# Cyan4973/FiniteStateEntropy

Measured on NVIDIA H100. Metric: encode+decode GB/s (uncompressed) per GPU on 32 KB blocks; bit-exact vs ref, higher is better.
Workload: dtype u8

## Files before the change

finitestateentropy_b200/csrc/huf_encode.cu:

```cuda
#include <cstdlib>
#include <mutex>
#include <type_traits>
#include <vector>
#include "common.cuh"
#include "launchers.h"
#include "launch_util.cuh"
#include "fse_dev.cuh"
#include "sink_dev.cuh"
#include "huf_build_dev.cuh"
#include "pack_dev.cuh"

namespace fseb {
namespace hufe {

constexpr unsigned FULL = 0xFFFFFFFFu;

struct __align__(16) Plan {
    u32 ctable[256];
    u8  header[136];
    u32 hSize;
    u32 state;
    u32 total;
    u32 streamOff[4];
    u32 streamBytes[4];
    u16 segCount[4][256];
};

constexpr int PLAN_WARPS = 8;
constexpr u32 GROUP = 32;
constexpr u32 HDR_STRIDE = 34 + 224 + 1;
constexpr u32 CT_ROW = HDR_STRIDE;
constexpr u32 ROWS = CT_ROW + 256;
constexpr u32 NODE_END = 0x7FFFFFFFu, LEAF_END = 0xFFFFFFFFu;
struct PlanCta {
    u32 nd[ROWS][GROUP];
    u8  sym[256][GROUP];
    u64 res[GROUP];
    u16 msv[GROUP];
    u8  last[GROUP];
    u8  tlog[GROUP];
    u8  live[GROUP];
};
static_assert(ROWS >= 1 + 256 + PLAN_WARPS * 4 * 256 / GROUP, "segment histograms must fit in the rows above the leaves");
static_assert(ROWS >= 1 + 511 && CT_ROW >= 1 + 256, "node rows");
static_assert(HUF_BLOCK_MAX < (1u << 24), "node counts share a word with an 8-bit parent / length");
static_assert(sizeof(PlanCta) <= 76 * 1024, "three CTAs per SM");

__device__ __forceinline__ void warp_hist_range(u32* cnt, const u8* s, u32 begin, u32 end, unsigned lane)
{
    u32 i = begin;
    u32 const head = min(end, (u32)((begin + 15) & ~15u));
    bool const vec = ((reinterpret_cast<u64>(s) & 15) == 0);
    if (vec) {
        for (u32 k = i + lane; k < head; k += 32) atomicAdd(&cnt[s[k]], 1u);
        i = head;
        u32 const nvec = (end - i) / 16;
        const uint4* const gv = reinterpret_cast<const uint4*>(s + i);
        for (u32 v0 = 0; v0 < nvec; v0 += 128) {
            uint4 x[4];
            #pragma unroll
            for (int h = 0; h < 4; h++) { u32 const vi = v0 + 32 * h + lane; x[h] = (vi < nvec) ? __ldg(gv + vi) : make_uint4(0, 0, 0, 0); }
            #pragma unroll
            for (int h = 0; h < 4; h++) {
                if (v0 + 32 * h + lane >= nvec) continue;
                u32 const wd[4] = { x[h].x, x[h].y, x[h].z, x[h].w };
                #pragma unroll
                for (int k = 0; k < 4; k++) {
                    u32 const y = wd[k];
                    atomicAdd(&cnt[y & 0xFF], 1u); atomicAdd(&cnt[__byte_perm(y, 0, 0x4441)], 1u);
                    atomicAdd(&cnt[__byte_perm(y, 0, 0x4442)], 1u); atomicAdd(&cnt[y >> 24], 1u);
                }
            }
        }
        i += nvec * 16;
    }
    for (u32 k = i + lane; k < end; k += 32) atomicAdd(&cnt[s[k]], 1u);
}

__device__ __forceinline__ void warp_hist4_pipelined(u32 (*count4)[256], const u8* s, u32 n, u32 seg, unsigned lane)
{
    const uint4* const gv = reinterpret_cast<const uint4*>(s) + lane;
    u32 const B = n / 2048, perSeg = seg / 2048;
    auto load = [&](uint4 (&x)[4], u32 b) {
        #pragma unroll
        for (int h = 0; h < 4; h++) x[h] = __ldg(gv + b * 128 + 32 * h);
    };
    auto count = [&](const uint4 (&x)[4], u32 b) {
        u32* const cnt = count4[b / perSeg];
        #pragma unroll
        for (int h = 0; h < 4; h++) {
            u32 const wd[4] = { x[h].x, x[h].y, x[h].z, x[h].w };
            #pragma unroll
            for (int k = 0; k < 4; k++) {
                u32 const y = wd[k];
                atomicAdd(&cnt[y & 0xFF], 1u); atomicAdd(&cnt[__byte_perm(y, 0, 0x4441)], 1u);
                atomicAdd(&cnt[__byte_perm(y, 0, 0x4442)], 1u); atomicAdd(&cnt[y >> 24], 1u);
            }
        }
    };
    uint4 xa[4], xb[4];
    load(xa, 0);
    #pragma unroll 1
    for (u32 b = 0; b < B; b += 2) {
        if (b + 1 < B) load(xb, b + 1);
        count(xa, b);
        if (b + 2 < B) load(xa, b + 2);
        if (b + 1 < B) count(xb, b + 1);
    }
}

template <class Geo, int NS>
__global__ void __launch_bounds__(32 * PLAN_WARPS, 3)
huf_plan_kernel(Geo g, u8* __restrict__ cbuf, u64* __restrict__ csizes, const u8* __restrict__ src,
                unsigned msvReq, unsigned tlogReq, Plan* __restrict__ plans)
{
    static_assert(NS == 4 || NS == 1, "4X or 1X");
    extern __shared__ __align__(16) unsigned char smem_raw[];
    PlanCta& S = *reinterpret_cast<PlanCta*>(smem_raw);
    unsigned const lane = threadIdx.x & 31u, warp = threadIdx.x >> 5;
    u32 const b0 = blockIdx.x * GROUP;
#define FSEB_FINAL(v) { if (lane == 0) { P.state = 1; enc_out(g, csizes, b) = (v); S.live[c] = 0; } continue; }

    u32 (*const count4)[256] = reinterpret_cast<u32 (*)[256]>(&S.nd[257][0] + warp * 4 * 256);
    #pragma unroll 1
    for (u32 c = warp; c < GROUP; c += PLAN_WARPS) {
        __syncwarp();
        u32 const b = b0 + c;
        if (b >= g.nBlocks) { if (lane == 0) S.live[c] = 0; continue; }
        u32 const n = enc_len(g, b);
        u64 const cap = enc_cap(g, b);
        const u8* const s = enc_src(g, src, b);
        Plan& P = plans[b];
        if (!n) FSEB_FINAL(0);
        if (!cap) FSEB_FINAL(0);
        if (n > HUF_BLOCK_MAX) FSEB_FINAL(err(E_SRC_WRONG));
        if (tlogReq > HUF_MAX_TLOG) FSEB_FINAL(err(E_TLOG_TOO_LARGE));
        if (msvReq > HUF_MAX_SV) FSEB_FINAL(err(E_MSV_TOO_LARGE));
        unsigned const msvDecl = msvReq ? msvReq : HUF_MAX_SV;

        u32 const seg = (n + 3) / 4;
        for (u32 i = lane; i < 4 * 256; i += 32) (&count4[0][0])[i] = 0;
        __syncwarp();
        if ((reinterpret_cast<u64>(s) & 15) == 0 && seg % 2048 == 0 && n == 4 * seg) warp_hist4_pipelined(count4, s, n, seg, lane);
        else {
            #pragma unroll 1
            for (u32 k = 0; k < 4; k++) {
                u32 const beg = min(k * seg, n), end = (k < 3) ? min((k + 1) * seg, n) : n;
                warp_hist_range(count4[k], s, beg, end, lane);
            }
        }
        __syncwarp();
        u32 cnt[8], top = 0, best = 0;
        #pragma unroll
        for (u32 i = 0; i < 8; i++) {
            u32 const sy = i * 32 + lane;
            cnt[i] = count4[0][sy] + count4[1][sy] + count4[2][sy] + count4[3][sy];
            if (cnt[i]) top = sy;
            best = max(best, cnt[i]);
        }
        #pragma unroll
        for (int dlt = 16; dlt; dlt >>= 1) { top = max(top, __shfl_xor_sync(FULL, top, dlt)); best = max(best, __shfl_xor_sync(FULL, best, dlt)); }
        if (msvDecl < 255 && top > msvDecl) FSEB_FINAL(err(E_MSV_TOO_SMALL));
        if (best == n) {
            if constexpr (!std::is_same_v<Geo, PackedDescs>) { if (lane == 0) enc_dst(g, cbuf, b)[0] = s[0]; }
            FSEB_FINAL(1);
        }
        if (best <= (n >> 7) + 4) FSEB_FINAL(0);
        u32 const msv = top;
        #pragma unroll
        for (u32 k = 0; k < 4; k++)
            #pragma unroll
            for (u32 i = 0; i < 8; i++) P.segCount[k][i * 32 + lane] = (u16)count4[k][i * 32 + lane];
        u32 key[8], nnz = 0;
        #pragma unroll
        for (u32 i = 0; i < 8; i++) { u32 const sy = i * 32 + lane; key[i] = ((sy <= msv ? cnt[i] : 0u) << 8) | (255u - sy); nnz += __popc(__ballot_sync(FULL, cnt[i] != 0)); }
        warp_sort256_desc(key, lane);
        #pragma unroll
        for (u32 i = 0; i < 8; i++) {
            u32 const r = i * 32 + lane;
            if (r <= msv) { S.nd[1 + r][c] = key[i] >> 8; S.sym[r][c] = (u8)(255u - (key[i] & 0xFFu)); }
        }
        if (lane == 0) {
            S.nd[0][c] = 0;
            S.msv[c] = (u16)msv; S.last[c] = (u8)(nnz - 1); S.live[c] = 1;
            S.tlog[c] = (u8)d_optimal_tablelog(tlogReq ? tlogReq : HUF_DEF_TLOG, n, msv, 1);
        }
    }
    __syncthreads();

    if (warp == 0) {
        u32 const c = lane;
        bool const live = S.live[c];
        u32 const msv = S.msv[c];
        u32* const col = &S.nd[1][c];
        auto at = [&](int i) -> u32& { return col[i * (int)GROUP]; };
        u32* const ct = &S.nd[CT_ROW][c];
        u64 res = 0;
        if (live) {
            int const last = S.last[c];
            int fresh = 256, leaf = last, inner = fresh;
            int const root = fresh + leaf - 1;
            {   u32 const x = at(leaf), y = at(leaf - 1);
                at(fresh) = x + y;
                fresh++; leaf -= 2;
            }
            u32 cl = leaf >= 0 ? at(leaf) : LEAF_END, ci = at(inner);
            while (fresh <= root) {
                int a, bb; u32 ca, cb;
                if (cl < ci) { a = leaf--; ca = cl; cl = leaf >= 0 ? at(leaf) : LEAF_END; } else { a = inner++; ca = ci; ci = inner < fresh ? at(inner) : NODE_END; }
                if (cl < ci) { bb = leaf--; cb = cl; cl = leaf >= 0 ? at(leaf) : LEAF_END; } else { bb = inner++; cb = ci; ci = inner < fresh ? at(inner) : NODE_END; }
                u32 const sum = ca + cb;
                at(fresh) = sum;
                if (inner == fresh) ci = sum;
                u32 const tag = (u32)(fresh - 256) << 24;
                at(a) = ca | tag; at(bb) = cb | tag;
                fresh++;
            }
            at(root) &= 0xFFFFFFu;
            for (int m = root - 1; m >= 256; m--) { u32 const v = at(m); at(m) = (v & 0xFFFFFFu) | (((at(256 + (int)(v >> 24)) >> 24) + 1) << 24); }
            for (int m = 0; m <= last; m++) { u32 const v = at(m); at(m) = (v & 0xFFFFFFu) | (((at(256 + (int)(v >> 24)) >> 24) + 1) << 24); }
            u32 const mb = d_huf_limit_depth(PackedNodeView{ col, (int)GROUP }, (u32)last, S.tlog[c]);
            if (mb > HUF_MAX_TLOG) res = err(E_GENERIC);
            else {
                u32 perLen[HUF_MAX_TLOG + 1], nextVal[HUF_MAX_TLOG + 1];
                for (u32 i = 0; i <= HUF_MAX_TLOG; i++) { perLen[i] = 0; nextVal[i] = 0; }
                for (int m = 0; m <= last; m++) perLen[at(m) >> 24]++;
                u32 v = 0;
                for (int m = (int)mb; m > 0; m--) { nextVal[m] = v; v = (v + perLen[m]) >> 1; }
                for (u32 r = 0; r <= msv; r++) ct[S.sym[r][c] * GROUP] = (int)r <= last ? at((int)r) >> 24 : 0u;
                for (u32 sy = 0; sy <= msv; sy++) { u32 const len = ct[sy * GROUP]; ct[sy * GROUP] = (nextVal[len]++ & 0xFFFF) | (len << 16); }
                S.tlog[c] = (u8)mb;
            }
        }
        __syncwarp();
        if (live && !is_err(res)) {
            u64 const cap = enc_cap(g, b0 + c);
            u32* const area = &S.nd[0][0] + c * HDR_STRIDE;
            struct Col { const u32* p; __device__ u32 operator[](u32 i) const { return p[i * GROUP]; } };
            res = d_huf_write_ctable(reinterpret_cast<u8*>(area), cap < 136 ? cap : 136, Col{ ct }, msv, S.tlog[c], area + 34);
        }
        S.res[c] = res;
    }
    __syncthreads();

    #pragma unroll 1
    for (u32 c = warp; c < GROUP; c += PLAN_WARPS) {
        if (!S.live[c]) continue;
        u32 const b = b0 + c;
        u32 const n = enc_len(g, b);
        u64 const cap = enc_cap(g, b);
        Plan& P = plans[b];
        u64 const hs = S.res[c];
        if (is_err(hs)) FSEB_FINAL(hs);
        if (hs + 12 >= n) FSEB_FINAL(0);
        u64 const capLeft = cap - hs;
        if (NS == 4 && (capLeft < 6 + 1 + 1 + 1 + 8 || n < 12)) FSEB_FINAL(0);
        u32 const msv = S.msv[c];
        u32 cell[8];
        #pragma unroll
        for (u32 i = 0; i < 8; i++) cell[i] = (i * 32 + lane <= msv) ? S.nd[CT_ROW + i * 32 + lane][c] : 0u;
        u32 bits[NS];
        #pragma unroll
        for (int k = 0; k < NS; k++) {
            u32 acc = 0;
            #pragma unroll
            for (u32 i = 0; i < 8; i++) {
                u32 const sy = i * 32 + lane;
                u32 const cnt = (NS == 4) ? (u32)P.segCount[k][sy]
                                          : (u32)P.segCount[0][sy] + P.segCount[1][sy] + P.segCount[2][sy] + P.segCount[3][sy];
                acc += cnt * (cell[i] >> 16);
            }
            #pragma unroll
            for (int dlt = 16; dlt; dlt >>= 1) acc += __shfl_xor_sync(FULL, acc, dlt);
            bits[k] = acc;
        }
        u64 op = (NS == 4) ? 6 : 0; bool fits = true;
        u32 offs[NS], lens[NS];
        #pragma unroll
        for (int t = 0; t < NS; t++) {
            u64 const capk = capLeft - op;
            u64 const tot = (u64)bits[t] + 1;
            if (fits && (capk <= 8 || (tot >> 3) >= capk - 8)) fits = false;
            offs[t] = (u32)(hs + op); lens[t] = (u32)((tot + 7) >> 3);
            op += lens[t];
        }
        u64 const total = hs + op;
        if (!fits || total >= (u64)n - 1) FSEB_FINAL(0);
        #pragma unroll
        for (u32 i = 0; i < 8; i++) P.ctable[i * 32 + lane] = cell[i];
        const u8* const hdr = reinterpret_cast<const u8*>(&S.nd[0][0] + c * HDR_STRIDE);
        for (u32 i = lane; i < (u32)hs; i += 32) P.header[i] = hdr[i];
        if (lane < NS) { P.streamOff[lane] = offs[lane]; P.streamBytes[lane] = lens[lane]; }
        if (lane == 0) { P.hSize = (u32)hs; P.state = 0; P.total = (u32)total; enc_out(g, csizes, b) = total; }
    }
#undef FSEB_FINAL
}

constexpr int THREADS = 128;

template <class Geo>
static __device__ __noinline__ void store_piece_exact(u32* gw, u32 j, uint4 v, u32 a0, u32 endByte)
{
    u32 const wd[4] = { v.x, v.y, v.z, v.w };
    u8* const pb = reinterpret_cast<u8*>(gw + j);
    for (u32 t = 0; t < 16; t++) { u32 const at = 4 * j + t; if (at >= a0 && at < endByte) pb[t] = (u8)(wd[t >> 2] >> (8 * (t & 3))); }
}

template <class Geo, int NS>
__global__ void __launch_bounds__(32 * NS)
huf_emit_kernel(Geo g, u8* __restrict__ cbuf, const u8* __restrict__ src, const Plan* __restrict__ plans, const u32* __restrict__ sharedCT)
{
    static_assert(NS == 4 || NS == 1, "4X or 1X");
    constexpr int NT = 32 * NS;
    constexpr u32 W = 512;
    __shared__ u32 ctab[256];
    constexpr u32 WP = W + 4;
    __shared__ __align__(16) u32 winAll[NS * WP];
    int const tid = threadIdx.x;
    unsigned const lane = tid & 31u; int const k = tid >> 5;
    u32 const b = blockIdx.x;
    const Plan& P = plans[b];
    if (P.state != 0) return;
    u32 const n = enc_len(g, b);
    const u8* const s = enc_src(g, src, b);
    u8* const d = enc_dst(g, cbuf, b);
    u32 const hSize = P.hSize, total = P.total;

    {   const u32* const ct = sharedCT ? sharedCT : P.ctable;
        if constexpr (NS == 4) {
            u32 const c0 = ct[tid], c1 = ct[tid + 128];
            ctab[tid] = (c0 >> 16) | (c0 << 8 & 0xFFFF00u); ctab[tid + 128] = (c1 >> 16) | (c1 << 8 & 0xFFFF00u);
        } else {
            #pragma unroll
            for (int i = tid; i < 256; i += NT) { u32 const c0 = ct[i]; ctab[i] = (c0 >> 16) | (c0 << 8 & 0xFFFF00u); }
        }
    }
    for (u32 i = tid; i < NS * WP; i += NT) winAll[i] = 0;
    for (u32 i = tid; i < hSize; i += NT) d[i] = P.header[i];
    if (NS == 4 && tid < 3) { u32 const v = P.streamBytes[tid]; d[hSize + 2 * tid] = (u8)v; d[hSize + 2 * tid + 1] = (u8)(v >> 8); }
    __syncthreads();
    {
        u32 const seg = (NS == 4) ? (n + 3) / 4 : n;
        int const segBeg = (int)(k * seg);
        int const segEnd = (k < NS - 1) ? (int)((k + 1) * seg) : (int)n;
        u32 sTab = (u32)__cvta_generic_to_shared(ctab);
        asm volatile("mov.u32 %0, %0;" : "+r"(sTab));
        u32* const win = winAll + k * WP;
        u32 sWin = (u32)__cvta_generic_to_shared(win);
        asm volatile("mov.u32 %0, %0;" : "+r"(sWin));
        u8* const gstart = d + P.streamOff[k];
        u32 const a0 = (u32)(reinterpret_cast<u64>(gstart) & 15);
        u32* const gw = reinterpret_cast<u32*>(gstart - a0);
        u32 const sBytes = (k < NS - 1) ? P.streamBytes[k] : total - P.streamOff[NS - 1];
        u32 const endByte = a0 + sBytes;
        u32 bitpos = 8u * a0;
        u32 flushed = 0;
        auto lds32 = [&](u32 a) -> u32 { u32 v; asm volatile("ld.shared.u32 %0, [%1];" : "=r"(v) : "r"(a)); return v; };
        auto lds64 = [&](u32 o) -> uint2 { u32 const e = lds32(sTab + (o >> 1)); return make_uint2(e >> 8, e & 0xFFu); };
        auto red_or = [&](u32 a, u32 v) { asm volatile("red.shared.or.b32 [%0], %1;" :: "r"(a), "r"(v) : "memory"); };
        auto red_or3 = [&](u32 a, u32 v0, u32 v1, u32 v2) {
            asm volatile("red.shared.or.b32 [%0], %1; red.shared.or.b32 [%0+4], %2; red.shared.or.b32 [%0+8], %3;" :: "r"(a), "r"(v0), "r"(v1), "r"(v2) : "memory");
        };
        auto scan = [&](u32 held, u32& excl) -> u32 {
            u32 incl = held;
            #pragma unroll
            for (int dd = 1; dd < 32; dd <<= 1)
                asm volatile("{ .reg .pred p; .reg .u32 t; shfl.sync.up.b32 t|p, %0, %1, 0, 0xffffffff; @p add.u32 %0, %0, t; }" : "+r"(incl) : "r"(dd));
            excl = incl - held;
            return __shfl_sync(FULL, incl, 31);
        };
        auto put = [&](u32 at, u32 x0, u32 x1) {
            u32 const sh = at & 31;
            red_or3(sWin + ((at >> 3) & (4 * (W - 1))), x0 << sh, __funnelshift_l(x0, x1, sh), __funnelshift_l(x1, 0, sh));
        };
        auto put96 = [&](u32 at, u32 z0, u32 z1, u32 z2) {
            u32 const sh = at & 31;
            asm volatile("red.shared.or.b32 [%0], %1; red.shared.or.b32 [%0+4], %2; red.shared.or.b32 [%0+8], %3; red.shared.or.b32 [%0+12], %4;"
                         :: "r"(sWin + ((at >> 3) & (4 * (W - 1)))), "r"(z0 << sh), "r"(__funnelshift_l(z0, z1, sh)), "r"(__funnelshift_l(z1, z2, sh)),
                            "r"(__funnelshift_l(z2, 0, sh)) : "memory");
        };
        auto flush = [&](bool all) {
            u32 const upTo = all ? (endByte + 3) / 4 : (bitpos >> 5);
            if (!all && flushed + 128 > upTo) return;
            __syncwarp();
            while (all ? flushed < upTo : flushed + 128 <= upTo) {
                u32 const j = flushed + 4 * lane;
                if (j < upTo) {
                    u32 const i = j & (W - 1);
                    uint4 v = *reinterpret_cast<uint4*>(win + i);
                    *reinterpret_cast<uint4*>(win + i) = make_uint4(0, 0, 0, 0);
                    if (i == 0) { v.x |= win[W]; v.y |= win[W + 1]; v.z |= win[W + 2]; win[W] = 0; win[W + 1] = 0; win[W + 2] = 0; }
                    if (!all && (j != 0 || a0 == 0)) *reinterpret_cast<uint4*>(gw + j) = v;
                    else store_piece_exact<Geo>(gw, j, v, a0, endByte);
                }
                flushed += 128;
            }
        };
        auto place = [&](u32 x0, u32 x1, u32 held) -> u32 {
            u32 excl; u32 const sum = scan(held, excl);
            put(bitpos + excl, x0, x1);
            return sum;
        };
        constexpr int PF = 4;
        int hiCur = segEnd;
        {
            bool const al8 = ((reinterpret_cast<u64>(s) + (u64)segEnd) & 7) == 0;
            int const nBig = al8 ? (segEnd - segBeg) / 256 : 0;
            const uint2* gq = reinterpret_cast<const uint2*>(s + segEnd) - 1 - lane;
            auto half = [&](u32 w, u32& a0, u32& a1) -> u32 {
                u32 const e0 = lds32(sTab + 4 * __byte_perm(w, 0, 0x4443)), e1 = lds32(sTab + 4 * __byte_perm(w, 0, 0x4442));
                u32 const e2 = lds32(sTab + 4 * __byte_perm(w, 0, 0x4441)), e3 = lds32(sTab + 4 * __byte_perm(w, 0, 0x4440));
                u32 const p01 = (e0 >> 8) | __funnelshift_l(0, e1 >> 8, e0), l01 = e0 + e1;
                u32 const p23 = (e2 >> 8) | __funnelshift_l(0, e3 >> 8, e2), l23 = e2 + e3;
                a0 = p01 | __funnelshift_l(0, p23, l01); a1 = __funnelshift_l(p23, 0, l01);
                return (l01 + l23) & 0xFFu;
            };
            auto merge = [&](u32 x0, u32 x1, u32 lx, u32 y0, u32 y1, u32& z0, u32& z1, u32& z2) {
                u32 const t0 = __funnelshift_l(0, y0, lx), t1 = __funnelshift_l(y0, y1, lx), t2 = __funnelshift_l(y1, 0, lx);
                bool const far = (lx & 32u) != 0;
                z0 = x0 | (far ? 0u : t0); z1 = x1 | (far ? t0 : t1); z2 = far ? t1 : t2;
            };
            auto big2 = [&](uint2 curA, uint2 curB) {
                u32 x0, x1, y0, y1, za0, za1, za2, zb0, zb1, zb2;
                u32 lx = half(curA.y, x0, x1), ly = half(curA.x, y0, y1);
                merge(x0, x1, lx, y0, y1, za0, za1, za2);
                u32 const la = lx + ly;
                lx = half(curB.y, x0, x1); ly = half(curB.x, y0, y1);
                merge(x0, x1, lx, y0, y1, zb0, zb1, zb2);
                u32 const lb = lx + ly;
                u32 excl; u32 const sum = scan(la | (lb << 16), excl);
                u32 const sumA = sum & 0xFFFFu;
                put96(bitpos + (excl & 0xFFFFu), za0, za1, za2);
                put96(bitpos + sumA + (excl >> 16), zb0, zb1, zb2);
                bitpos += sumA + (sum >> 16);
                flush(false);
            };
            constexpr int PB = 2;
            int const rounds = nBig / PB;
            uint2 bufA[PB], bufB[PB];
            #pragma unroll
            for (int i = 0; i < PB; i++) { bufA[i] = rounds > 0 ? __ldg(gq - 32 * i) : make_uint2(0, 0); bufB[i] = make_uint2(0, 0); }
            auto round = [&](uint2 (&X)[PB], uint2 (&Y)[PB], int r) {
                gq -= 32 * PB;
                uint2 const c0 = X[0], c1 = X[1];
                if (r + 1 < rounds) { Y[0] = __ldg(gq); Y[1] = __ldg(gq - 32); }
                big2(c0, c1);
            };
            int r = 0;
            #pragma unroll 1
            for (; r + 1 < rounds; r += 2) { round(bufA, bufB, r); round(bufB, bufA, r + 1); }
            if (r < rounds) round(bufA, bufB, r);
            hiCur -= 256 * rounds * PB;
        }
        bool const wordAligned = ((reinterpret_cast<u64>(s) + (u64)hiCur) & 3) == 0;
        int const nFull = wordAligned ? (hiCur - segBeg) / 128 : 0;
        {
            const u32* gp = reinterpret_cast<const u32*>(s + hiCur) - 1 - lane;
            auto group = [&](u32 o0, u32 o1, u32 o2, u32 o3) {
                uint2 const e0 = lds64(o0), e1 = lds64(o1), e2 = lds64(o2), e3 = lds64(o3);
                u32 const p01 = e0.x | (e1.x << e0.y), l01 = e0.y + e1.y;
                u32 const p23 = e2.x | (e3.x << e2.y), l23 = e2.y + e3.y;
                u32 const a0 = p01 | (p23 << l01), a1 = __funnelshift_l(p23, 0, l01);
                bitpos += place(a0, a1, l01 + l23);
                flush(false);
            };
            int const rounds = nFull / PF;
            u32 bufA[PF], bufB[PF];
            #pragma unroll
            for (int i = 0; i < PF; i++) { bufA[i] = rounds > 0 ? __ldg(gp - 32 * i) : 0u; bufB[i] = 0u; }
            auto round = [&](u32 (&X)[PF], u32 (&Y)[PF], int r) {
                gp -= 32 * PF;
                bool const more = r + 1 < rounds;
                #pragma unroll
                for (int i = 0; i < PF; i++) {
                    u32 const cur = X[i];
                    if (more) Y[i] = __ldg(gp - 32 * i);
                    group(8 * (cur >> 24), 8 * __byte_perm(cur, 0, 0x4442), 8 * __byte_perm(cur, 0, 0x4441), 8 * (cur & 0xFFu));
                }
            };
            int r = 0;
            #pragma unroll 1
            for (; r + 1 < rounds; r += 2) { round(bufA, bufB, r); round(bufB, bufA, r + 1); }
            if (r < rounds) round(bufA, bufB, r);
            for (int j = rounds * PF; j < nFull; j++) {
                u32 const cur = __ldg(reinterpret_cast<const u32*>(s + hiCur) - 1 - lane - 32 * j);
                group(8 * (cur >> 24), 8 * __byte_perm(cur, 0, 0x4442), 8 * __byte_perm(cur, 0, 0x4441), 8 * (cur & 0xFFu));
            }
        }
        {
            int const rest = hiCur - 128 * nFull;
            auto fetch = [&](int hi) -> u32 {
                int const top = hi - 4 * (int)lane;
                u32 v = 0;
                if (top - 4 >= segBeg && ((reinterpret_cast<u64>(s + top) & 3) == 0)) v = __ldg(reinterpret_cast<const u32*>(s + top - 4));
                else if (top > segBeg) {
                    #pragma unroll
                    for (int j = 0; j < 4; j++) { int const i = top - 1 - j; if (i >= segBeg) v |= (u32)s[i] << (8 * (3 - j)); }
                }
                return v;
            };
            #pragma unroll 1
            for (int hi = rest; hi > segBeg; hi -= 128) {
                u32 const cur = fetch(hi);
                int const nValid = hi - 4 * (int)lane - segBeg;
                u64 acc = 0; u32 held = 0;
                #pragma unroll
                for (int j = 0; j < 4; j++) {
                    uint2 const e = lds64(8 * ((cur >> (8 * (3 - j))) & 0xFF));
                    if (j < nValid) { acc |= (u64)e.x << held; held += e.y; }
                }
                bitpos += place((u32)acc, (u32)(acc >> 32), held);
                flush(false);
            }
        }
        if (lane == 0) red_or(sWin + 4 * ((bitpos >> 5) & (W - 1)), 1u << (bitpos & 31));
        bitpos += 1;
        flush(true);
    }
}

struct HufPlace {
    typedef PackedDescs Geo;
    typedef Plan* Aux;
    static __device__ __forceinline__ u64 value(const PackedDescs& g, u64 b) { return g.result[b]; }
    static __device__ __forceinline__ u64 len(const PackedDescs& g, u64 b, u64 v) { return packed_len(v, g.srcSize[b]); }
    static __device__ __forceinline__ void place(const PackedDescs& g, Plan* plans, u64 b, u64 v, u64 off, u64 len)
    {
        g.offset[b] = off;
        if (!is_err(v) && off + len > g.outCap) { g.result[b] = err(E_DST_TOO_SMALL); plans[b].state = 1; }
        else if (v == 1) g.out[off] = g.src[b][0];
    }
};

__global__ void __launch_bounds__(pack::COPY_THREADS)
huf_pack_raw_kernel(PackedDescs g)
{
    u32 const b = blockIdx.x;
    if (g.result[b] != 0) return;
    u32 const n = (u32)g.srcSize[b];
    if (n == 0) return;
    const u8* const s = g.src[b];
    u8* const d = g.out + g.offset[b];
    pack::cta_copy<pack::COPY_THREADS, pack::COPY_UNROLL>(d, s, n);
}

__global__ void __launch_bounds__(32 * PLAN_WARPS)
huf_sizes_kernel(BatchGeom g, u64* __restrict__ csizes, const u8* __restrict__ src, const u32* __restrict__ ct, Plan* __restrict__ plans)
{
    __shared__ u8 nbOf[256];
    unsigned const lane = threadIdx.x & 31u;
    for (u32 i = threadIdx.x; i < 256; i += blockDim.x) nbOf[i] = (u8)(ct[i] >> 16);
    __syncthreads();
    u32 const b = blockIdx.x * PLAN_WARPS + (threadIdx.x >> 5);
    if (b >= g.nBlocks) return;
    u32 const n = block_len(g, b);
    const u8* const s = src + (u64)b * g.blockSize;
    u64 const cap = g.slot;
    Plan& P = plans[b];
    if (cap < 6 + 1 + 1 + 1 + 8 || n < 12) { if (lane == 0) { P.state = 1; csizes[b] = 0; } return; }
    u32 const seg = (n + 3) / 4;
    u32 bits[4];
    #pragma unroll 1
    for (u32 k = 0; k < 4; k++) {
        u32 const beg = k * seg, end = (k < 3) ? (k + 1) * seg : n;
        u32 acc = 0;
        u32 i = beg + lane * 4;
        if ((reinterpret_cast<u64>(s + beg) & 3) == 0) {
            for (; i + 4 <= end; i += 128) {
                u32 const w = __ldg(reinterpret_cast<const u32*>(s + i));
                acc += nbOf[w & 0xFF] + nbOf[(w >> 8) & 0xFF] + nbOf[(w >> 16) & 0xFF] + nbOf[w >> 24];
            }
            for (u32 t = i; t < end && t < i + 4; t++) acc += nbOf[s[t]];
        } else for (u32 t = beg + lane; t < end; t += 32) acc += nbOf[s[t]];
        #pragma unroll
        for (int dlt = 16; dlt; dlt >>= 1) acc += __shfl_xor_sync(FULL, acc, dlt);
        bits[k] = acc;
    }
    u64 op = 6; bool fits = true;
    u32 offs[4], lens[4];
    #pragma unroll
    for (int t = 0; t < 4; t++) {
        u64 const capk = cap - op;
        u64 const tot = (u64)bits[t] + 1;
        if (fits && (capk <= 8 || (tot >> 3) >= capk - 8)) fits = false;
        offs[t] = (u32)op; lens[t] = (u32)((tot + 7) >> 3);
        op += lens[t];
    }
    if (!fits) { if (lane == 0) { P.state = 1; csizes[b] = 0; } return; }
    if (lane < 4) { P.streamOff[lane] = offs[lane]; P.streamBytes[lane] = lens[lane]; }
    if (lane == 0) { P.hSize = 0; P.state = 0; P.total = (u32)op; csizes[b] = op; }
}

}

cudaError_t launch_huf_encode_using_ctable(const BatchGeom& g, void* cbuf, u64* csizes, const void* src, const u32* dCTable, cudaStream_t stream)
{
    if (g.nBlocks == 0) return cudaSuccess;
    cudaError_t e;
    hufe::Plan* const plans = (hufe::Plan*)stream_scratch(2, stream, sizeof(hufe::Plan) * (size_t)g.nBlocks, &e);
    if (e != cudaSuccess) return e;
    unsigned const grid = (g.nBlocks + hufe::PLAN_WARPS - 1) / hufe::PLAN_WARPS;
    hufe::huf_sizes_kernel<<<grid, 32 * hufe::PLAN_WARPS, 0, stream>>>(g, csizes, (const u8*)src, dCTable, plans);
    hufe::huf_emit_kernel<BatchGeom, 4><<<g.nBlocks, hufe::THREADS, 0, stream>>>(g, (u8*)cbuf, (const u8*)src, plans, dCTable);
    return cudaGetLastError();
}

namespace {
struct SubBatch { BatchGeom g; u8* cbuf; const u8* src; };
SubBatch sub_batch(const BatchGeom& g, u8* cbuf, const u8* src, u32 b0, u32 n)
{
    BatchGeom gs = g;
    gs.nBlocks = n;
    u64 const off = (u64)b0 * g.blockSize;
    u64 const span = (u64)n * g.blockSize;
    gs.total = (g.total - off < span) ? g.total - off : span;
    return { gs, cbuf + (u64)b0 * g.slot, src + off };
}
struct SubDescs { BlockDescs g; u8* cbuf; const u8* src; };
SubDescs sub_batch(const BlockDescs& g, u8*, const u8*, u32 b0, u32 n) { return { slice(g, b0, n), nullptr, nullptr }; }
struct SubPacked { PackedDescs g; u8* cbuf; const u8* src; };
SubPacked sub_batch(const PackedDescs& g, u8*, const u8*, u32 b0, u32 n) { return { slice(g, b0, n), nullptr, nullptr }; }

template <class Geo, int NS>
cudaError_t huf_encode(const Geo& g, void* cbuf, u64* csizes, const void* src, unsigned msv, unsigned tlog, cudaStream_t stream)
{
    if (g.nBlocks == 0) return cudaSuccess;
    cudaError_t e;
    hufe::Plan* plans = nullptr;
    static int asyncScratch = -1;
    if (asyncScratch < 0) { const char* const v = getenv("FSEB200_SCRATCH_ASYNC"); asyncScratch = (v && atoi(v) == 1) ? 1 : 0; }
    size_t const need = sizeof(hufe::Plan) * (size_t)g.nBlocks;
    if (asyncScratch) e = cudaMallocAsync((void**)&plans, need, stream);
    else plans = (hufe::Plan*)stream_scratch(2, stream, need, &e);
    if (e != cudaSuccess) return e;
    static u32 const subBatch = [] { const char* const v = getenv("FSEB200_HUF_ENC_SUBBATCH"); long n = v ? atol(v) : 0; return (u32)(n < 0 ? 0 : n); }();
    size_t const smem = sizeof(hufe::PlanCta);
    static SmemOptIn optin;
    e = optin.ensure(hufe::huf_plan_kernel<Geo, NS>, current_device(), (int)smem);
    if (e != cudaSuccess) return e;
    u32 const step = (subBatch && subBatch < g.nBlocks) ? subBatch : g.nBlocks;
    constexpr bool packed = std::is_same_v<Geo, PackedDescs>;
    u64* tileSum = nullptr;
    if constexpr (packed) {
        tileSum = (u64*)stream_scratch(4, stream, sizeof(u64) * pack::tiles_of(step), &e);
        if (e != cudaSuccess) { if (asyncScratch) cudaFreeAsync(plans, stream); return e; }
    }
    for (u32 b0 = 0; b0 < g.nBlocks; b0 += step) {
        auto const sb = sub_batch(g, (u8*)cbuf, (const u8*)src, b0, (g.nBlocks - b0 < step) ? g.nBlocks - b0 : step);
        u64* const cs = csizes ? csizes + b0 : nullptr;
        unsigned const grid = (sb.g.nBlocks + hufe::GROUP - 1) / hufe::GROUP;
        hufe::huf_plan_kernel<Geo, NS><<<grid, 32 * hufe::PLAN_WARPS, smem, stream>>>(sb.g, sb.cbuf, cs, sb.src, msv, tlog, plans + b0);
        if constexpr (packed) {
            pack::launch_pack<hufe::HufPlace>(sb.g, tileSum, b0 ? sb.g.offset : nullptr, sb.g.offset + sb.g.nBlocks, plans + b0, stream);
            hufe::huf_pack_raw_kernel<<<sb.g.nBlocks, pack::COPY_THREADS, 0, stream>>>(sb.g);
        }
        hufe::huf_emit_kernel<Geo, NS><<<sb.g.nBlocks, 32 * NS, 0, stream>>>(sb.g, sb.cbuf, sb.src, plans + b0, nullptr);
    }
    e = cudaGetLastError();
    cudaError_t const e2 = asyncScratch ? cudaFreeAsync(plans, stream) : cudaSuccess;
    return e != cudaSuccess ? e : e2;
}
}

cudaError_t launch_huf_encode(const BatchGeom& g, void* cbuf, u64* csizes, const void* src,
                              unsigned msv, unsigned tlog, cudaStream_t stream)
{
    return huf_encode<BatchGeom, 4>(g, cbuf, csizes, src, msv, tlog, stream);
}

cudaError_t launch_huf_encode_blocks(const BlockDescs& g, int nStreams, unsigned msv, unsigned tlog, cudaStream_t stream)
{
    return nStreams == 1 ? huf_encode<BlockDescs, 1>(g, nullptr, nullptr, nullptr, msv, tlog, stream)
                         : huf_encode<BlockDescs, 4>(g, nullptr, nullptr, nullptr, msv, tlog, stream);
}

cudaError_t launch_huf_encode_packed(const PackedDescs& g, int nStreams, unsigned msv, unsigned tlog, cudaStream_t stream)
{
    return nStreams == 1 ? huf_encode<PackedDescs, 1>(g, nullptr, nullptr, nullptr, msv, tlog, stream)
                         : huf_encode<PackedDescs, 4>(g, nullptr, nullptr, nullptr, msv, tlog, stream);
}

}
```

finitestateentropy_b200/csrc/launch_util.cuh:

```cuda
#pragma once
#include <cuda_runtime.h>
#include <mutex>
#include <vector>

namespace fseb {

constexpr int MAX_DEVICES = 64;

inline int current_device()
{
    int dev = 0;
    if (cudaGetDevice(&dev) != cudaSuccess || dev < 0 || dev >= MAX_DEVICES) dev = 0;
    return dev;
}

inline int device_sm_count(int dev)
{
    static int sms[MAX_DEVICES];
    static std::once_flag once[MAX_DEVICES];
    std::call_once(once[dev], [dev] {
        int n = 132;
        if (cudaDeviceGetAttribute(&n, cudaDevAttrMultiProcessorCount, dev) != cudaSuccess || n <= 0) n = 132;
        sms[dev] = n;
    });
    return sms[dev];
}

inline int device_smem_optin(int dev)
{
    static int bytes[MAX_DEVICES];
    static std::once_flag once[MAX_DEVICES];
    std::call_once(once[dev], [dev] {
        int n = 0;
        if (cudaDeviceGetAttribute(&n, cudaDevAttrMaxSharedMemoryPerBlockOptin, dev) != cudaSuccess || n < 0) n = 0;
        bytes[dev] = n;
    });
    return bytes[dev];
}

struct SmemOptIn {
    std::mutex mu;
    int granted[MAX_DEVICES] = {};
    template <typename K>
    cudaError_t ensure(K kernel, int dev, int bytes)
    {
        std::lock_guard<std::mutex> lock(mu);
        if (granted[dev] >= bytes) return cudaSuccess;
        cudaError_t const e = cudaFuncSetAttribute(kernel, cudaFuncAttributeMaxDynamicSharedMemorySize, bytes);
        if (e == cudaSuccess) granted[dev] = bytes;
        return e;
    }
};

inline void* stream_scratch(int purpose, cudaStream_t stream, size_t bytes, cudaError_t* err)
{
    struct Slot { int purpose, dev; cudaStream_t s; void* p; size_t cap; };
    static std::mutex mu;
    static std::vector<Slot> slots;
    std::lock_guard<std::mutex> lock(mu);
    int const dev = current_device();
    Slot* hit = nullptr;
    for (auto& sl : slots) if (sl.purpose == purpose && sl.s == stream && sl.dev == dev) { hit = &sl; break; }
    if (!hit) { slots.push_back(Slot{ purpose, dev, stream, nullptr, 0 }); hit = &slots.back(); }
    *err = cudaSuccess;
    if (hit->cap < bytes) {
        if (hit->p) { cudaStreamSynchronize(stream); cudaFree(hit->p); hit->p = nullptr; hit->cap = 0; }
        *err = cudaMalloc(&hit->p, bytes);
        if (*err != cudaSuccess) return nullptr;
        hit->cap = bytes;
    }
    return hit->p;
}

}
```

Measured before the change: 415.5.

## Overlap Huffman emit with plan kernel via PDL and per-group ready flags

Launches the emit kernel as a programmatic dependent launch so it can begin while the plan kernel is still running. Each plan CTA publishes an epoch-tagged ready flag with release semantics, and each emit CTA spins with acquire loads and nanosleep backoff until its group's flag is set. This hides launch latency and the tail gap between the two kernels, at the cost of spin-waiting CTAs that occupy SM slots, plus a per-stream epoch scratch buffer. It applies only to the non-packed path.

Measured after the change: 421.1, median of 6. 1.01x the previous value.

```diff
diff --git a/finitestateentropy_b200/csrc/huf_encode.cu b/finitestateentropy_b200/csrc/huf_encode.cu
--- a/finitestateentropy_b200/csrc/huf_encode.cu
+++ b/finitestateentropy_b200/csrc/huf_encode.cu
@@ -109,12 +109,31 @@
     }
 }
 
+__device__ __forceinline__ void publish_group(u32* flag, u32 epoch)
+{
+    __threadfence();
+    asm volatile("st.release.gpu.global.u32 [%0], %1;" :: "l"(flag), "r"(epoch) : "memory");
+}
+
+__device__ __forceinline__ void await_group(const u32* flag, u32 epoch)
+{
+    u32 ns = 32;
+    for (;;) {
+        u32 v;
+        asm volatile("ld.acquire.gpu.global.u32 %0, [%1];" : "=r"(v) : "l"(flag) : "memory");
+        if (v == epoch) return;
+        __nanosleep(ns);
+        ns = ns < 1024 ? 2 * ns : ns;
+    }
+}
+
 template <class Geo, int NS>
 __global__ void __launch_bounds__(32 * PLAN_WARPS, 3)
 huf_plan_kernel(Geo g, u8* __restrict__ cbuf, u64* __restrict__ csizes, const u8* __restrict__ src,
-                unsigned msvReq, unsigned tlogReq, Plan* __restrict__ plans)
+                unsigned msvReq, unsigned tlogReq, Plan* __restrict__ plans, u32* __restrict__ ready, u32 epoch)
 {
     static_assert(NS == 4 || NS == 1, "4X or 1X");
+    asm volatile("griddepcontrol.launch_dependents;");
     extern __shared__ __align__(16) unsigned char smem_raw[];
     PlanCta& S = *reinterpret_cast<PlanCta*>(smem_raw);
     unsigned const lane = threadIdx.x & 31u, warp = threadIdx.x >> 5;
@@ -294,6 +313,10 @@
         if (lane == 0) { P.hSize = (u32)hs; P.state = 0; P.total = (u32)total; enc_out(g, csizes, b) = total; }
     }
 #undef FSEB_FINAL
+    if (ready) {
+        __syncthreads();
+        if (threadIdx.x == 0) publish_group(ready + blockIdx.x, epoch);
+    }
 }
 
 constexpr int THREADS = 128;
@@ -308,7 +331,8 @@
 
 template <class Geo, int NS>
 __global__ void __launch_bounds__(32 * NS)
-huf_emit_kernel(Geo g, u8* __restrict__ cbuf, const u8* __restrict__ src, const Plan* __restrict__ plans, const u32* __restrict__ sharedCT)
+huf_emit_kernel(Geo g, u8* __restrict__ cbuf, const u8* __restrict__ src, const Plan* plans, const u32* __restrict__ sharedCT,
+                const u32* ready, u32 epoch)
 {
     static_assert(NS == 4 || NS == 1, "4X or 1X");
     constexpr int NT = 32 * NS;
@@ -319,6 +343,10 @@
     int const tid = threadIdx.x;
     unsigned const lane = tid & 31u; int const k = tid >> 5;
     u32 const b = blockIdx.x;
+    if (ready) {
+        if (tid == 0) await_group(ready + b / GROUP, epoch);
+        __syncthreads();
+    }
     const Plan& P = plans[b];
     if (P.state != 0) return;
     u32 const n = enc_len(g, b);
@@ -601,7 +629,7 @@
     if (e != cudaSuccess) return e;
     unsigned const grid = (g.nBlocks + hufe::PLAN_WARPS - 1) / hufe::PLAN_WARPS;
     hufe::huf_sizes_kernel<<<grid, 32 * hufe::PLAN_WARPS, 0, stream>>>(g, csizes, (const u8*)src, dCTable, plans);
-    hufe::huf_emit_kernel<BatchGeom, 4><<<g.nBlocks, hufe::THREADS, 0, stream>>>(g, (u8*)cbuf, (const u8*)src, plans, dCTable);
+    hufe::huf_emit_kernel<BatchGeom, 4><<<g.nBlocks, hufe::THREADS, 0, stream>>>(g, (u8*)cbuf, (const u8*)src, plans, dCTable, nullptr, 0);
     return cudaGetLastError();
 }
 
@@ -641,22 +669,35 @@
     u32 const step = (subBatch && subBatch < g.nBlocks) ? subBatch : g.nBlocks;
     constexpr bool packed = std::is_same_v<Geo, PackedDescs>;
     u64* tileSum = nullptr;
+    u32* ready = nullptr;
+    u32 epoch = 0;
+    auto groups_of = [](u32 n) { return (n + hufe::GROUP - 1) / hufe::GROUP; };
     if constexpr (packed) {
         tileSum = (u64*)stream_scratch(4, stream, sizeof(u64) * pack::tiles_of(step), &e);
-        if (e != cudaSuccess) { if (asyncScratch) cudaFreeAsync(plans, stream); return e; }
-    }
-    for (u32 b0 = 0; b0 < g.nBlocks; b0 += step) {
+    } else {
+        u32 const groups = (g.nBlocks / step) * groups_of(step) + groups_of(g.nBlocks % step);
+        ready = (u32*)stream_scratch(9, stream, sizeof(u32) * groups, &e, &epoch);
+    }
+    if (e != cudaSuccess) { if (asyncScratch) cudaFreeAsync(plans, stream); return e; }
+    u32 group0 = 0;
+    for (u32 b0 = 0; b0 < g.nBlocks && e == cudaSuccess; b0 += step) {
         auto const sb = sub_batch(g, (u8*)cbuf, (const u8*)src, b0, (g.nBlocks - b0 < step) ? g.nBlocks - b0 : step);
         u64* const cs = csizes ? csizes + b0 : nullptr;
-        unsigned const grid = (sb.g.nBlocks + hufe::GROUP - 1) / hufe::GROUP;
-        hufe::huf_plan_kernel<Geo, NS><<<grid, 32 * hufe::PLAN_WARPS, smem, stream>>>(sb.g, sb.cbuf, cs, sb.src, msv, tlog, plans + b0);
+        unsigned const grid = groups_of(sb.g.nBlocks);
+        u32* const rdy = packed ? nullptr : ready + group0;
+        hufe::huf_plan_kernel<Geo, NS><<<grid, 32 * hufe::PLAN_WARPS, smem, stream>>>(sb.g, sb.cbuf, cs, sb.src, msv, tlog, plans + b0, rdy, epoch);
+        group0 += grid;
         if constexpr (packed) {
             pack::launch_pack<hufe::HufPlace>(sb.g, tileSum, b0 ? sb.g.offset : nullptr, sb.g.offset + sb.g.nBlocks, plans + b0, stream);
             hufe::huf_pack_raw_kernel<<<sb.g.nBlocks, pack::COPY_THREADS, 0, stream>>>(sb.g);
-        }
-        hufe::huf_emit_kernel<Geo, NS><<<sb.g.nBlocks, 32 * NS, 0, stream>>>(sb.g, sb.cbuf, sb.src, plans + b0, nullptr);
-    }
-    e = cudaGetLastError();
+            hufe::huf_emit_kernel<Geo, NS><<<sb.g.nBlocks, 32 * NS, 0, stream>>>(sb.g, sb.cbuf, sb.src, plans + b0, nullptr, nullptr, 0);
+        } else {
+            e = launch_dependent(hufe::huf_emit_kernel<Geo, NS>, sb.g.nBlocks, 32 * NS, 0, stream, sb.g, sb.cbuf, sb.src, plans + b0,
+                                 nullptr, rdy, epoch);
+        }
+    }
+    cudaError_t const le = cudaGetLastError();
+    if (e == cudaSuccess) e = le;
     cudaError_t const e2 = asyncScratch ? cudaFreeAsync(plans, stream) : cudaSuccess;
     return e != cudaSuccess ? e : e2;
 }
diff --git a/finitestateentropy_b200/csrc/launch_util.cuh b/finitestateentropy_b200/csrc/launch_util.cuh
--- a/finitestateentropy_b200/csrc/launch_util.cuh
+++ b/finitestateentropy_b200/csrc/launch_util.cuh
@@ -52,22 +52,43 @@
     }
 };
 
-inline void* stream_scratch(int purpose, cudaStream_t stream, size_t bytes, cudaError_t* err)
+template <typename... P, typename... A>
+cudaError_t launch_dependent(void (*kernel)(P...), unsigned grid, unsigned threads, size_t smem, cudaStream_t stream, A... args)
 {
-    struct Slot { int purpose, dev; cudaStream_t s; void* p; size_t cap; };
+    cudaLaunchAttribute attr[1];
+    attr[0].id = cudaLaunchAttributeProgrammaticStreamSerialization;
+    attr[0].val.programmaticStreamSerializationAllowed = 1;
+    cudaLaunchConfig_t cfg = {};
+    cfg.gridDim = dim3(grid); cfg.blockDim = dim3(threads); cfg.dynamicSmemBytes = smem; cfg.stream = stream;
+    cfg.attrs = attr; cfg.numAttrs = 1;
+    return cudaLaunchKernelEx(&cfg, kernel, static_cast<P>(args)...);
+}
+
+inline void* stream_scratch(int purpose, cudaStream_t stream, size_t bytes, cudaError_t* err, unsigned* epoch = nullptr)
+{
+    struct Slot { int purpose, dev; cudaStream_t s; void* p; size_t cap; unsigned epoch; };
     static std::mutex mu;
     static std::vector<Slot> slots;
     std::lock_guard<std::mutex> lock(mu);
     int const dev = current_device();
     Slot* hit = nullptr;
     for (auto& sl : slots) if (sl.purpose == purpose && sl.s == stream && sl.dev == dev) { hit = &sl; break; }
-    if (!hit) { slots.push_back(Slot{ purpose, dev, stream, nullptr, 0 }); hit = &slots.back(); }
+    if (!hit) { slots.push_back(Slot{ purpose, dev, stream, nullptr, 0, 0 }); hit = &slots.back(); }
     *err = cudaSuccess;
     if (hit->cap < bytes) {
         if (hit->p) { cudaStreamSynchronize(stream); cudaFree(hit->p); hit->p = nullptr; hit->cap = 0; }
+        hit->epoch = 0;
         *err = cudaMalloc(&hit->p, bytes);
         if (*err != cudaSuccess) return nullptr;
         hit->cap = bytes;
+    }
+    if (epoch) {
+        if (hit->epoch == 0 || hit->epoch == ~0u) {
+            *err = cudaMemsetAsync(hit->p, 0, hit->cap, stream);
+            if (*err != cudaSuccess) return nullptr;
+            hit->epoch = 0;
+        }
+        *epoch = ++hit->epoch;
     }
     return hit->p;
 }
```
